# notu97/GS-SLAM-Analytica_Jacobian

Measured on AMD Instinct MI355X. Metric: Gaussian-pixel interactions/sec (fwd+Jacobian), 640x480, higher is better.
Workload: dtype f32; 1 GPU; cfg2: 50000 Gaussians (SH degree 3, 16 coeffs), 640x480; one step = one mapping window of 8 keyframes with distinct cameras: forward splat + analytical-Jacobian backward (dL/dmu, dL/dSigma->conic, per-Gaussian grads summed over the window, one dL/dtau per keyframe)

## Files before the change

gs-slam-analytica_jacobian_amd/csrc/api.hip:

```cpp
#include <stdarg.h>
#include <stdio.h>
#include <string.h>

#include <atomic>
#include <mutex>

#include "gsaj_common.h"
#include "loss_terms.h"

static thread_local char g_err[512] = "";

void gsaj_set_error(const char *fmt, ...) {
  va_list ap;
  va_start(ap, fmt);
  vsnprintf(g_err, sizeof(g_err), fmt, ap);
  va_end(ap);
}

struct ProfRec { int stage; hipEvent_t a, b; };
static std::mutex g_prof_mu;
static ProfRec *g_prof = nullptr;
static std::atomic<bool> g_prof_on{false};
static int g_prof_cap = 0;
static std::atomic<int> g_prof_n{0};
static thread_local int t_prof_open = -1;

void gsaj_prof_mark(int stage, int is_stop, hipStream_t s) {
  if (!g_prof_on.load(std::memory_order_acquire)) return;
  std::lock_guard<std::mutex> lk(g_prof_mu);
  if (!g_prof) return;
  if (!is_stop) {
    const int i = g_prof_n.fetch_add(1);
    if (i >= g_prof_cap) { g_prof_n.store(g_prof_cap); t_prof_open = -1; return; }
    t_prof_open = i;
    g_prof[i].stage = stage;
    (void)hipEventRecord(g_prof[i].a, s);
  } else if (t_prof_open >= 0 && t_prof_open < g_prof_cap) {
    (void)hipEventRecord(g_prof[t_prof_open].b, s);
    t_prof_open = -1;
  }
}

extern "C" {

int gsaj_profile_begin(int max_records) {
  std::lock_guard<std::mutex> lk(g_prof_mu);
  if (g_prof || max_records <= 0) {
    gsaj_set_error("gsaj_profile_begin: already active or bad size");
    return GSAJ_ERR_INVALID_ARGUMENT;
  }
  g_prof = new ProfRec[max_records];
  for (int i = 0; i < max_records; i++) {
    GSAJ_HIP_CHECK(hipEventCreate(&g_prof[i].a));
    GSAJ_HIP_CHECK(hipEventCreate(&g_prof[i].b));
  }
  g_prof_cap = max_records;
  g_prof_n.store(0);
  g_prof_on.store(true, std::memory_order_release);
  return GSAJ_OK;
}

int gsaj_profile_end(float *stage_ms, int *stage_launches) {
  if (!stage_ms || !stage_launches) {
    gsaj_set_error("gsaj_profile_end: null output");
    return GSAJ_ERR_INVALID_ARGUMENT;
  }
  g_prof_on.store(false, std::memory_order_release);
  GSAJ_HIP_CHECK(hipDeviceSynchronize());
  std::lock_guard<std::mutex> lk(g_prof_mu);
  if (!g_prof) {
    gsaj_set_error("gsaj_profile_end: not active");
    return GSAJ_ERR_INVALID_ARGUMENT;
  }
  for (int i = 0; i < ST_COUNT; i++) { stage_ms[i] = 0.f; stage_launches[i] = 0; }
  const int nrec = g_prof_n.load() < g_prof_cap ? g_prof_n.load() : g_prof_cap;
  for (int i = 0; i < nrec; i++) {
    float ms = 0.f;
    if (hipEventElapsedTime(&ms, g_prof[i].a, g_prof[i].b) == hipSuccess) {
      stage_ms[g_prof[i].stage] += ms;
      stage_launches[g_prof[i].stage] += 1;
    }
  }
  for (int i = 0; i < g_prof_cap; i++) { (void)hipEventDestroy(g_prof[i].a); (void)hipEventDestroy(g_prof[i].b); }
  delete[] g_prof;
  g_prof = nullptr;
  g_prof_cap = 0;
  g_prof_n.store(0);
  return GSAJ_OK;
}

const char *gsaj_last_error(void) { return g_err; }
int gsaj_version(void) { return 109; }

size_t gsaj_geom_workspace_bytes(int P) { return geom_carve(nullptr, (size_t)(P > 0 ? P : 0), nullptr) + 256; }
size_t gsaj_image_workspace_bytes(int W, int H) { return image_carve(nullptr, W, H, nullptr) + 256; }
size_t gsaj_binning_workspace_bytes(int R) {
  return bin_carve(nullptr, (size_t)(R > 0 ? R : 0), nullptr) + 256;
}

// ... 849 lines not shown
```

gs-slam-analytica_jacobian_amd/csrc/gaussian_bwd.hip:

```cpp
#include "gsaj_common.h"
#include "wave_reduce.h"
__constant__ float bSH_C0 = 0.28209479177387814f;
__constant__ float bSH_C1 = 0.4886025119029199f;
__constant__ float bSH_C2[5] = {1.0925484305920792f, -1.0925484305920792f, 0.31539156525252005f, -1.0925484305920792f,
                                0.5462742152960396f};
__constant__ float bSH_C3[7] = {-0.5900435899266435f, 2.890611442640554f, -0.4570457994644658f, 0.3731763325901154f,
                                -0.4570457994644658f, 1.445305721320277f, -0.5900435899266435f};
#define GSAJ_SH_CONSTANTS_DEFINED
#include "gaussian_chain.h"

__device__ __forceinline__ void gsaj_load_partials4(const float *p0, const float *p1, const float *p2, const float *p3,
                                                    float4 (&lo)[4], float4 (&hi)[4]) {
  asm volatile(
      "global_load_dwordx4 %0, %8, off sc0 sc1\n\tglobal_load_dwordx4 %1, %8, off offset:16 sc0 sc1\n\t"
      "global_load_dwordx4 %2, %9, off sc0 sc1\n\tglobal_load_dwordx4 %3, %9, off offset:16 sc0 sc1\n\t"
      "global_load_dwordx4 %4, %10, off sc0 sc1\n\tglobal_load_dwordx4 %5, %10, off offset:16 sc0 sc1\n\t"
      "global_load_dwordx4 %6, %11, off sc0 sc1\n\tglobal_load_dwordx4 %7, %11, off offset:16 sc0 sc1\n\t"
      "s_waitcnt vmcnt(0)"
      : "=&v"(lo[0]), "=&v"(hi[0]), "=&v"(lo[1]), "=&v"(hi[1]), "=&v"(lo[2]), "=&v"(hi[2]), "=&v"(lo[3]), "=&v"(hi[3])
      : "v"(p0), "v"(p1), "v"(p2), "v"(p3)
      : "memory");
}
__device__ __forceinline__ void gsaj_sum_partials(const float *partials, int nblk, int lane, double (&acc)[6]) {
  for (int i0 = lane; i0 < nblk; i0 += 4 * 64) {
// ... 540 lines not shown
        t6[k] = wave_sum<CW_G>(tau[k]);
      }
      if (gl == 0) {
        float4 *tp = reinterpret_cast<float4 *>(g.tau_partials + (size_t)blockIdx.x * 8);
        tp[0] = make_float4(t6[0], t6[1], t6[2], t6[3]);
        tp[1] = make_float4(t6[4], t6[5], 0.f, 0.f);
      }
    }
    float *mine = rowv + vl * NV * CW_G + gl;
    mine[0 * CW_G] = o.op; mine[1 * CW_G] = o.gm.x; mine[2 * CW_G] = o.gm.y; mine[3 * CW_G] = o.gm.z;
#pragma unroll
    for (int k = 0; k < 6; k++) mine[(4 + k) * CW_G] = o.cov[k];
    if constexpr (GATHER && SHW > 0) {
      if (!sh_left) {
        mine[10 * CW_G] = 0.f; mine[11 * CW_G] = 0.f; mine[12 * CW_G] = 0.f;
#pragma unroll
        for (int k = 0; k < MC; k++) mine[(13 + k) * CW_G] = 0.f;
      }
    } else {
      mine[10 * CW_G] = gmask.x; mine[11 * CW_G] = gmask.y; mine[12 * CW_G] = gmask.z;
#pragma unroll
      for (int k = 0; k < MC; k++) mine[(13 + k) * CW_G] = w[k];
    }
    __syncthreads();
    const int nv = min(CW_V, K - v0);
#pragma unroll
    for (int j = 0; j < EPT; j++) {
      const int e = tid + j * (CW_G * CW_V);
      const int c = e / CW_G;
      if (c < NE) {
        float sacc = acc[j];
        if (c < 10) {
#pragma unroll 2
          for (int u = 0; u < nv; u++) sacc += rowv[u * NV * CW_G + c * CW_G + gl];
        } else {
          const int kk = (c - 10) / 3, ch = (c - 10) - 3 * kk;
#pragma unroll 2
          for (int u = 0; u < nv; u++) sacc += rowv[u * NV * CW_G + (13 + kk) * CW_G + gl] * rowv[u * NV * CW_G + (10 + ch) * CW_G + gl];
        }
        acc[j] = sacc;
      }
    }
    __syncthreads();
  }
#pragma unroll
  for (int j = 0; j < EPT; j++) {
    const int e = tid + j * (CW_G * CW_V);
    if (e < NE * CW_G) outv[e] = acc[j];
  }
  __syncthreads();
#define OUT(dst, x) dst = accumulate ? dst + (x) : (x)
  const int nG = min(CW_G, p.P - (int)blockIdx.x * CW_G);
  const size_t b0 = (size_t)blockIdx.x * CW_G;
  for (int e = tid; e < nG; e += CW_G * CW_V) OUT(p.dL_dopacity[b0 + e], outv[0 * CW_G + e]);
  for (int e = tid; e < 3 * nG; e += CW_G * CW_V) OUT(p.dL_dmean3D[3 * b0 + e], outv[(1 + e % 3) * CW_G + e / 3]);
  for (int e = tid; e < 6 * nG; e += CW_G * CW_V) OUT(p.dL_dcov3D[6 * b0 + e], outv[(4 + e % 6) * CW_G + e / 6]);
  if (SHW > 0 && p.dL_dsh) {
    for (int e = tid; e < SHW * nG; e += CW_G * CW_V) OUT(p.dL_dsh[(size_t)SHW * b0 + e], outv[(10 + e % SHW) * CW_G + e / SHW]);
  }
  if (p.scales && tid < nG) {
    const size_t i = b0 + tid;
    float gcov[6];
#pragma unroll
    for (int k = 0; k < 6; k++) gcov[k] = outv[(4 + k) * CW_G + tid];
    const float3 sc = make_float3(p.scales[3 * i], p.scales[3 * i + 1], p.scales[3 * i + 2]);
    const float4 q = reinterpret_cast<const float4 *>(p.rotations)[i];
    float3 dscale;
    float4 drot;
    cov3d_backward(gcov, sc, q, p.scale_modifier, dscale, drot);
    OUT(p.dL_dscale[3 * i], dscale.x); OUT(p.dL_dscale[3 * i + 1], dscale.y); OUT(p.dL_dscale[3 * i + 2], dscale.z);
    float4 *dr = reinterpret_cast<float4 *>(p.dL_drot) + i;
    if (accumulate) { const float4 o4 = *dr; drot.x += o4.x; drot.y += o4.y; drot.z += o4.z; drot.w += o4.w; }
    *dr = drot;
  }
#undef OUT
  GSAJ_TRACE_END(gbb)
}

__global__ __launch_bounds__(256) void k_tau_sum(BwdParams p, GeomWS g0, ViewStrides vs) {
  __shared__ double red[256 * 6];
  const int tid = threadIdx.x, view = blockIdx.x, nslot = (p.P + CW_G - 1) / CW_G;
  const float4 *tp = reinterpret_cast<const float4 *>(gsaj_shift(g0.tau_partials, (size_t)view * vs.geom));
  double a[6] = {0.0, 0.0, 0.0, 0.0, 0.0, 0.0};
  for (int i = tid; i < nslot; i += 256) {
    const float4 lo = tp[2 * i], hi = tp[2 * i + 1];
    a[0] += (double)lo.x; a[1] += (double)lo.y; a[2] += (double)lo.z; a[3] += (double)lo.w; a[4] += (double)hi.x; a[5] += (double)hi.y;
  }
#pragma unroll
  for (int k = 0; k < 6; k++) red[k * 256 + tid] = a[k];
  __syncthreads();
  for (int o = 128; o > 0; o >>= 1) {
    if (tid < o) {
#pragma unroll
      for (int k = 0; k < 6; k++) red[k * 256 + tid] += red[k * 256 + tid + o];
    }
    __syncthreads();
  }
  if (tid < 6 && p.dL_dtau_sum) p.dL_dtau_sum[6 * view + tid] = (float)red[tid * 256];
}

template <int SHW, bool GATHER>
static void launch_chain(const BwdParams &p, int K, const GeomWS &g, const BinWS &b, const ImageWS &im, ViewStrides vs, int accumulate,
                         hipStream_t s) {
  for (int v0 = 0; v0 < K; v0 += CW_V)
    hipLaunchKernelGGL((k_chain_window<SHW, GATHER>), dim3((p.P + CW_G - 1) / CW_G), dim3(CW_G * CW_V), 0, s, p, v0, K, g, im, vs,
                       b.inst_grad, b.reached, p.dL_dmean2D, p.dL_dconic, p.dL_dcolor, p.dL_ddepth, p.dL_dtau,
                       (accumulate || v0 > 0) ? 1 : 0);
  hipLaunchKernelGGL(k_tau_sum, dim3(K), dim3(256), 0, s, p, g, vs);
}

int launch_gather_sums(int P, int K, const int *radii, const GeomWS &g, const BinWS &b, const ImageWS &im, ViewStrides vs, hipStream_t s) {
  GsajProfScope ps(ST_GATHER_SUMS, s);
  hipLaunchKernelGGL(k_gather_sums, dim3((P + 255) / 256, K), dim3(256), 0, s, P, radii, g, im, b.inst_grad, b.reached, vs);
  GSAJ_HIP_CHECK(hipGetLastError());
  return GSAJ_OK;
}

int launch_gaussian_backward_batch(const BwdParams &p, int K, const GeomWS &g, const BinWS &b, const ImageWS &im, ViewStrides vs,
                                   int accumulate, int gather, hipStream_t s) {
  GsajProfScope ps(ST_GAUSSIAN_BWD, s);
#define CHAIN(SHW)                                                       \
  if (gather) launch_chain<SHW, true>(p, K, g, b, im, vs, accumulate, s); \
  else launch_chain<SHW, false>(p, K, g, b, im, vs, accumulate, s);       \
  break
  switch (p.shs ? p.M : 0) {
    case 0: CHAIN(0);
    case 1: CHAIN(3);
    case 4: CHAIN(12);
    case 9: CHAIN(27);
    case 16: CHAIN(48);
    default:
      gsaj_set_error("batched backward: SH storage of %d coefficients is not supported (1, 4, 9 or 16)", p.M);
      return GSAJ_ERR_INVALID_ARGUMENT;
  }
#undef CHAIN
  GSAJ_HIP_CHECK(hipGetLastError());
  return GSAJ_OK;
}
```

gs-slam-analytica_jacobian_amd/csrc/gsaj_common.h:

```cpp
#pragma once
#include <hip/hip_runtime.h>
#include <stddef.h>
#include <stdint.h>

#include "../../include/gsaj.h"

#define GSAJ_WAVE 64
#define TILE GSAJ_TILE
#define TILE_PIXELS (TILE * TILE)
#define PRE_BLOCK 256
#define GB_BLOCK 64
#define REC_F4 3
#define IGRAD_F 12


static inline __host__ __device__ size_t gsaj_align(size_t x) { return (x + 255) & ~(size_t)255; }

struct GeomWS {
  float *depths;
  float *cov3D;
  uint8_t *clamped;
  uint32_t *tiles_touched;
  uint32_t *point_offsets;
  int *internal_radii;
  uint32_t *block_sums;
  float *tau_partials;
  float4 *splat;
  float4 *splat16;
  uint2 *scat;
  float4 *gsum;
};

static inline __host__ __device__ size_t geom_carve(char *base, size_t P, GeomWS *g) {
  size_t off = 0;
  size_t nblk = (P + PRE_BLOCK - 1) / PRE_BLOCK;
  if (nblk == 0) nblk = 1;
#define CARVE(field, type, count)                                \
  do {                                                           \
    if (g) g->field = reinterpret_cast<type *>(base + off);      \
    off += gsaj_align(sizeof(type) * (size_t)(count));           \
  } while (0)
  CARVE(depths, float, P);
  CARVE(cov3D, float, P * 6);
  CARVE(clamped, uint8_t, P * 3);
  CARVE(tiles_touched, uint32_t, P);
  CARVE(point_offsets, uint32_t, P);
  CARVE(internal_radii, int, P);
  CARVE(block_sums, uint32_t, nblk);
  CARVE(tau_partials, float, ((P + 31) / 32 + 1) * 8);
  CARVE(splat, float4, P * 3);
  CARVE(splat16, float4, P * 2);
  CARVE(scat, uint2, P);
  CARVE(gsum, float4, P * 3);
  return off;
}

#define TILE_REP 1
#define LDS_TILES_MAX 8192
#define SORT_CAP 16384
#define N_COUNTERS 64
#define ERR_PREFILTERED 1u
#define ERR_INTERNAL 2u
#define ERR_CAPACITY 4u
#define ERR_TILE_LIST 8u

struct ImageWS {
  float *final_T;
  uint32_t *n_contrib;
  uint2 *ranges;
  uint32_t *counters;
  uint32_t *tile_count;
  uint32_t *tile_cursor;
  uint32_t *tile_offset;
  uint32_t *sticky;
  uint32_t *tile_order;
  size_t zero_bytes;
};

static inline __host__ __device__ size_t image_carve(char *base, int W, int H, ImageWS *s) {
  size_t off = 0;
  size_t N = (size_t)W * H;
  size_t tiles = (size_t)((W + TILE - 1) / TILE) * ((H + TILE - 1) / TILE);
  ImageWS *g = s;
  CARVE(final_T, float, N);
  CARVE(n_contrib, uint32_t, N);
  CARVE(ranges, uint2, tiles);
  const size_t z0 = off;
  CARVE(counters, uint32_t, N_COUNTERS);
  CARVE(tile_count, uint32_t, tiles * TILE_REP);
  CARVE(tile_cursor, uint32_t, tiles * TILE_REP);
  if (g) g->zero_bytes = off - z0;
  CARVE(tile_offset, uint32_t, tiles * TILE_REP + 1);
  CARVE(sticky, uint32_t, 16);
  CARVE(tile_order, uint32_t, tiles);
  return off;
}

struct BinWS {
  uint64_t *keys_unsorted;
  uint64_t *keys;
  uint32_t *point_list;
  float4 *inst_grad;
  uint8_t *reached;
  uint32_t *taken;
};

struct ViewStrides {
  size_t geom, image, bin;
};
#ifdef __HIPCC__
#include <type_traits>
template <typename T>
__device__ __forceinline__ T *gsaj_shift(T *p, size_t bytes) {
  typedef typename std::conditional<std::is_const<T>::value, const char, char>::type byte_t;
  return reinterpret_cast<T *>(reinterpret_cast<byte_t *>(p) + bytes);
}
__device__ __forceinline__ GeomWS geom_view(GeomWS g, size_t off) {
  g.depths = gsaj_shift(g.depths, off); g.cov3D = gsaj_shift(g.cov3D, off); g.clamped = gsaj_shift(g.clamped, off);
  g.tiles_touched = gsaj_shift(g.tiles_touched, off); g.point_offsets = gsaj_shift(g.point_offsets, off);
  g.internal_radii = gsaj_shift(g.internal_radii, off); g.block_sums = gsaj_shift(g.block_sums, off);
  g.tau_partials = gsaj_shift(g.tau_partials, off); g.splat = gsaj_shift(g.splat, off); g.gsum = gsaj_shift(g.gsum, off);
  g.splat16 = gsaj_shift(g.splat16, off); g.scat = gsaj_shift(g.scat, off);
  return g;
}
__device__ __forceinline__ ImageWS image_view(ImageWS m, size_t off) {
  m.final_T = gsaj_shift(m.final_T, off); m.n_contrib = gsaj_shift(m.n_contrib, off); m.ranges = gsaj_shift(m.ranges, off);
  m.counters = gsaj_shift(m.counters, off); m.tile_count = gsaj_shift(m.tile_count, off);
  m.tile_cursor = gsaj_shift(m.tile_cursor, off); m.tile_offset = gsaj_shift(m.tile_offset, off);
  m.sticky = gsaj_shift(m.sticky, off); m.tile_order = gsaj_shift(m.tile_order, off);
  return m;
}
#endif

static inline size_t bin_carve(char *base, size_t R, BinWS *g) {
  size_t off = 0;
  size_t Rn = R ? R : 1;
  CARVE(keys_unsorted, uint64_t, Rn);
  CARVE(keys, uint64_t, Rn);
  CARVE(point_list, uint32_t, Rn);
  CARVE(inst_grad, float4, Rn * REC_F4);
  CARVE(reached, uint8_t, Rn);
  CARVE(taken, uint32_t, Rn);
  return off;
}
#undef CARVE

struct Carved { GeomWS g; BinWS b; ImageWS im; ViewStrides vs; };

void gsaj_set_error(const char *fmt, ...);
#define GSAJ_HIP_CHECK(expr)                                                          \
  do {                                                                                \
    hipError_t _e = (expr);                                                           \
    if (_e != hipSuccess) {                                                           \
      gsaj_set_error("%s failed: %s (%s:%d)", #expr, hipGetErrorString(_e), __FILE__, __LINE__); \
      return GSAJ_ERR_HIP;                                                            \
    }                                                                                 \
  } while (0)

enum GsajStage {
  ST_PREPROCESS = 0, ST_SCAN, ST_EMIT_KEYS, ST_SORT, ST_RANGES_RECORDS, ST_RENDER_FWD, ST_RENDER_BWD, ST_GAUSSIAN_BWD,
  ST_TAU_FINALIZE, ST_DENSE_BWD, ST_DENSE_REDUCE, ST_SCATTER, ST_TILE_SORT, ST_GATHER_SUMS, ST_COUNT
};
void gsaj_prof_mark(int stage, int is_stop, hipStream_t s);
struct GsajProfScope {
  int stage;
  hipStream_t s;
  GsajProfScope(int st, hipStream_t stream) : stage(st), s(stream) { gsaj_prof_mark(stage, 0, s); }
  ~GsajProfScope() { gsaj_prof_mark(stage, 1, s); }
};

struct FwdParams {
  int P, D, M, W, H;
  const float *means3D, *shs, *colors_precomp, *opacities, *scales, *rotations, *cov3D_precomp;
  const float *viewmatrix, *projmatrix, *campos;
  float scale_modifier, tanfovx, tanfovy, focal_x, focal_y;
  int prefiltered;
  int grid_x, grid_y;
  int capacity;
  int sort_cap;
  int bpw;
  int views;
};

int launch_preprocess(const FwdParams &p, int *radii, int *n_touched, const GeomWS &g, const ImageWS &im, ViewStrides vs,
                      hipStream_t s);
int launch_tile_binning(int P, int sort_cap, int rec16, int grid_x, int grid_y, const GeomWS &g, const BinWS &b, const ImageWS &im,
                        int views, ViewStrides vs, hipStream_t s);
struct FusedLoss;
int launch_render_forward(int P, int W, int H, int grid_x, int grid_y, const float *bg, const GeomWS &g, const BinWS &b,
                          const ImageWS &im, float *out_color, float *out_depth, float *out_opacity, int *n_touched, int views,
                          ViewStrides vs, hipStream_t s, const FusedLoss *fl = nullptr);
int gsaj_fwd_loss_slots(int W, int H);
int launch_loss_finalize(const FusedLoss &fl, int nslots, int W, int H, const uint32_t *aborted, float *out_scalars, hipStream_t s,
                         int views = 1, size_t abort_stride = 0, float *out_dexposure = nullptr);
int launch_render_backward(int R, int W, int H, int grid_x, int grid_y, const float *bg, const GeomWS &g, const BinWS &b,
                           const ImageWS &im, const float *dL_dpix, const float *dL_dpix_depth, int views, ViewStrides vs,
                           hipStream_t s, const FusedLoss *fl = nullptr);
int launch_export_taken(int W, int H, int grid_x, int grid_y, const BinWS &b, const ImageWS &im, uint32_t *out, hipStream_t s);
struct BwdParams {
  int P, D, M, W, H;
  const float *means3D, *shs, *scales, *rotations, *cov3Ds;
  const float *viewmatrix, *projmatrix, *projmatrix_raw, *campos;
  float scale_modifier, tanfovx, tanfovy, focal_x, focal_y;
  int grid_x, grid_y;
  const int *radii;
  float *dL_dmean2D, *dL_dconic, *dL_dopacity, *dL_dcolor, *dL_ddepth, *dL_dmean3D, *dL_dcov3D, *dL_dsh, *dL_dscale,
      *dL_drot, *dL_dtau, *dL_dtau_sum;
};
int launch_gaussian_backward(const BwdParams &p, const GeomWS &g, const BinWS &b, const ImageWS &im, hipStream_t s);
int launch_gather_sums(int P, int K, const int *radii, const GeomWS &g, const BinWS &b, const ImageWS &im, ViewStrides vs, hipStream_t s);
int launch_gaussian_backward_batch(const BwdParams &p, int K, const GeomWS &g, const BinWS &b, const ImageWS &im, ViewStrides vs,
                                   int accumulate, int gather, hipStream_t s);
size_t gsaj_jac_rows_bytes(int P);
int gsaj_jac_slots(int W, int H);
int launch_splat_jac(const BwdParams &p, const GeomWS &g, const ImageWS &im, float *rows, hipStream_t s);
struct JacOut {
  float *jac;
  float *color, *depth;
  const float *seed_c, *seed_d;
  const float *curv_c, *curv_d;
  float *partials;
  float delta;
};
int launch_render_jac(const BwdParams &p, const float *bg, const GeomWS &g, const BinWS &b, const ImageWS &im, const float *rows,
                      const JacOut &jo, const FusedLoss *fl, int joint, hipStream_t s);
int launch_gn_reduce(const float *partials, int n, const ImageWS &im, float *H_out, float *g_out, hipStream_t s);
int launch_splat_jac_batch(const BwdParams &p, int K, const GeomWS &g, const ImageWS &im, float *rows, ViewStrides vs, hipStream_t s);
int launch_render_jac_batch(const BwdParams &p, int K, const float *bg, const Carved &c, const float *rows, const JacOut &jo,
                            const FusedLoss &fl, int joint, hipStream_t s);
int launch_mark_visible(int P, const float *means3D, const float *viewmatrix, uint8_t *present, hipStream_t s);
void launch_exclusive_scan_u32(int n, uint32_t *v, hipStream_t s);
int launch_select_rank_f32(int W, int H, const float *values, uint32_t rank, uint32_t *out_key, void *seed_ws, hipStream_t s);

#ifdef __HIPCC__
__device__ __forceinline__ float3 xform4x3(const float *m, float3 p) {
  return make_float3(m[0] * p.x + m[4] * p.y + m[8] * p.z + m[12], m[1] * p.x + m[5] * p.y + m[9] * p.z + m[13],
                     m[2] * p.x + m[6] * p.y + m[10] * p.z + m[14]);
}
__device__ __forceinline__ float4 xform4x4(const float *m, float3 p) {
  return make_float4(m[0] * p.x + m[4] * p.y + m[8] * p.z + m[12], m[1] * p.x + m[5] * p.y + m[9] * p.z + m[13],
                     m[2] * p.x + m[6] * p.y + m[10] * p.z + m[14], m[3] * p.x + m[7] * p.y + m[11] * p.z + m[15]);
}
__device__ __forceinline__ float ndc2pix(float v, int S) { return (float)((((double)v + 1.0) * (double)S - 1.0) * 0.5); }

__device__ __forceinline__ uint32_t gsaj_tile_band(const uint32_t *__restrict__ sticky) {
  const uint32_t band = sticky[1];
  return sticky[2] == ~band ? band : 0u;
}
__device__ __forceinline__ void tile_rect(float px, float py, int r, int gx, int gy, uint32_t band, int &x0, int &y0, int &x1,
                                          int &y1) {
  const int ylo = band ? (int)(band & 0xffffu) : 0, yhi = band ? min(gy, (int)(band >> 16)) : gy;
  x0 = min(gx, max(0, (int)((px - (float)r) / (float)TILE)));
// ... 116 lines not shown
```

gs-slam-analytica_jacobian_amd/csrc/preprocess.hip:

```cpp
#include "gsaj_common.h"
#include "wave_reduce.h"

__constant__ float kSH_C0 = 0.28209479177387814f;
__constant__ float kSH_C1 = 0.4886025119029199f;
__constant__ float kSH_C2[5] = {1.0925484305920792f, -1.0925484305920792f, 0.31539156525252005f, -1.0925484305920792f,
                                0.5462742152960396f};
__constant__ float kSH_C3[7] = {-0.5900435899266435f, 2.890611442640554f, -0.4570457994644658f, 0.3731763325901154f,
                                -0.4570457994644658f, 1.445305721320277f, -0.5900435899266435f};

__device__ __forceinline__ float3 ld3(const float *p, size_t i) { return make_float3(p[3 * i], p[3 * i + 1], p[3 * i + 2]); }

__device__ __forceinline__ void cov3d_from_scale_rot(float3 sc, float mod, float4 q, float *c6) {
  const float r = q.x, x = q.y, y = q.z, z = q.w;
  float R[3][3] = {{1.f - 2.f * (y * y + z * z), 2.f * (x * y - r * z), 2.f * (x * z + r * y)},
                   {2.f * (x * y + r * z), 1.f - 2.f * (x * x + z * z), 2.f * (y * z - r * x)},
                   {2.f * (x * z - r * y), 2.f * (y * z + r * x), 1.f - 2.f * (x * x + y * y)}};
  const float s[3] = {mod * sc.x, mod * sc.y, mod * sc.z};
  float A[3][3];
#pragma unroll
  for (int i = 0; i < 3; i++)
#pragma unroll
    for (int j = 0; j < 3; j++) A[i][j] = s[i] * R[j][i];
  float S[3][3];
#pragma unroll
  for (int a = 0; a < 3; a++)
#pragma unroll
    for (int b = a; b < 3; b++) S[a][b] = A[0][a] * A[0][b] + A[1][a] * A[1][b] + A[2][a] * A[2][b];
  c6[0] = S[0][0]; c6[1] = S[0][1]; c6[2] = S[0][2]; c6[3] = S[1][1]; c6[4] = S[1][2]; c6[5] = S[2][2];
}

__device__ __forceinline__ float3 cov2d_forward(float3 mean, float fx, float fy, float tanx, float tany, const float *c6,
                                                const float *vm) {
  float3 t = xform4x3(vm, mean);
  const float limx = 1.3f * tanx, limy = 1.3f * tany;
  const float txtz = t.x / t.z, tytz = t.y / t.z;
  t.x = fminf(limx, fmaxf(-limx, txtz)) * t.z;
  t.y = fminf(limy, fmaxf(-limy, tytz)) * t.z;
  const float J00 = fx / t.z, J02 = -(fx * t.x) / (t.z * t.z);
  const float J11 = fy / t.z, J12 = -(fy * t.y) / (t.z * t.z);
  float M[2][3];
#pragma unroll
  for (int k = 0; k < 3; k++) {
    M[0][k] = vm[4 * k + 0] * J00 + vm[4 * k + 1] * 0.0f + vm[4 * k + 2] * J02;
    M[1][k] = vm[4 * k + 0] * 0.0f + vm[4 * k + 1] * J11 + vm[4 * k + 2] * J12;
  }
  const float V[3][3] = {{c6[0], c6[1], c6[2]}, {c6[1], c6[3], c6[4]}, {c6[2], c6[4], c6[5]}};
  float X[2][3];
#pragma unroll
  for (int r = 0; r < 2; r++)
#pragma unroll
    for (int c = 0; c < 3; c++) X[r][c] = M[r][0] * V[c][0] + M[r][1] * V[c][1] + M[r][2] * V[c][2];
  float3 cov;
  cov.x = (X[0][0] * M[0][0] + X[0][1] * M[0][1] + X[0][2] * M[0][2]) + 0.3f;
  cov.y = X[1][0] * M[0][0] + X[1][1] * M[0][1] + X[1][2] * M[0][2];
  cov.z = (X[1][0] * M[1][0] + X[1][1] * M[1][1] + X[1][2] * M[1][2]) + 0.3f;
  return cov;
}

__device__ __forceinline__ float3 sh_to_rgb(int deg, float3 pos, float3 campos, const float *sh, uint8_t *clamped) {
  float3 d = make_float3(pos.x - campos.x, pos.y - campos.y, pos.z - campos.z);
  const float len = sqrtf(d.x * d.x + d.y * d.y + d.z * d.z);
  const float x = d.x / len, y = d.y / len, z = d.z / len;
  float out[3];
#pragma unroll
  for (int ch = 0; ch < 3; ch++) {
#define SHC(k) sh[(k) * 3 + ch]
    float res = kSH_C0 * SHC(0);
    if (deg > 0) {
      res = res - kSH_C1 * y * SHC(1) + kSH_C1 * z * SHC(2) - kSH_C1 * x * SHC(3);
      if (deg > 1) {
        const float xx = x * x, yy = y * y, zz = z * z, xy = x * y, yz = y * z, xz = x * z;
        res = res + kSH_C2[0] * xy * SHC(4) + kSH_C2[1] * yz * SHC(5) + kSH_C2[2] * (2.0f * zz - xx - yy) * SHC(6) +
              kSH_C2[3] * xz * SHC(7) + kSH_C2[4] * (xx - yy) * SHC(8);
        if (deg > 2) {
          res = res + kSH_C3[0] * y * (3.0f * xx - yy) * SHC(9) + kSH_C3[1] * xy * z * SHC(10) +
                kSH_C3[2] * y * (4.0f * zz - xx - yy) * SHC(11) + kSH_C3[3] * z * (2.0f * zz - 3.0f * xx - 3.0f * yy) * SHC(12) +
                kSH_C3[4] * x * (4.0f * zz - xx - yy) * SHC(13) + kSH_C3[5] * z * (xx - yy) * SHC(14) +
                kSH_C3[6] * x * (xx - 3.0f * yy) * SHC(15);
        }
      }
    }
#undef SHC
    res += 0.5f;
    clamped[ch] = (res < 0.0f);
    out[ch] = res < 0.0f ? 0.0f : res;
  }
  return make_float3(out[0], out[1], out[2]);
}

GSAJ_TRACE_DEFINE(pre)

template <bool SH16, bool MULTI>
__global__ __launch_bounds__(PRE_BLOCK) void k_preprocess(FwdParams p, int *__restrict__ radii, int *__restrict__ n_touched,
                                                         GeomWS g, ImageWS im, ViewStrides vs) {
  __shared__ uint32_t scan[PRE_BLOCK / 64];
  extern __shared__ uint32_t hist[];
  {
    const size_t view = blockIdx.y;
    g = geom_view(g, view * vs.geom);
    im = image_view(im, view * vs.image);
    p.viewmatrix += 16 * view;
    p.projmatrix += 16 * view;
    if (p.campos) p.campos += 3 * view;
    radii += view * (size_t)p.P;
    n_touched += view * (size_t)p.P;
  }
  GSAJ_TRACE_BEGIN(pre)
#ifdef GSAJ_BLOCK_TRACE
  unsigned long long trp_[4] = {0, 0, 0, 0}, trp_t = wall_clock64();
#define TRP(i) { const unsigned long long n_ = wall_clock64(); trp_[i] += n_ - trp_t; trp_t = n_; }
#else
#define TRP(i)
#endif
  const int tid = threadIdx.x;
  const int tiles = p.grid_x * p.grid_y;
  const bool use_lds = tiles <= LDS_TILES_MAX;
  if (use_lds) {
    for (int t = tid; t < tiles; t += PRE_BLOCK) hist[t] = 0u;
    __syncthreads();
  }
  const int nblk_all = (p.P + PRE_BLOCK - 1) / PRE_BLOCK;
#pragma clang loop unroll(disable)
  for (int it = 0; it < (MULTI ? p.bpw : 1); it++) {
  const int blk = MULTI ? (int)blockIdx.x * p.bpw + it : (int)blockIdx.x;
  if (blk >= nblk_all) break;
  const int idx = blk * PRE_BLOCK + tid;
  uint32_t touched = 0;
  uint32_t rect_x = 0, rect_y = 0;
  float depth = 0.f;
  if (idx < p.P) {
    int my_radius_i = 0;
    uint32_t rect_pack = 0;
    float2 xy = make_float2(0.f, 0.f);
    float4 con_o = make_float4(0.f, 0.f, 0.f, 0.f);
    float3 rgb = make_float3(0.f, 0.f, 0.f);
    uint8_t cl[3] = {0, 0, 0};
    float c6s[6] = {0.f, 0.f, 0.f, 0.f, 0.f, 0.f};
    const float3 p_orig = ld3(p.means3D, idx);
    float3 sc_in = make_float3(0.f, 0.f, 0.f);
    float4 q_in = make_float4(1.f, 0.f, 0.f, 0.f);
    if (!p.cov3D_precomp) {
      sc_in = ld3(p.scales, idx);
      q_in = reinterpret_cast<const float4 *>(p.rotations)[idx];
    }
    const float opac_in = p.opacities[idx];
    constexpr bool sh_regs = SH16;
    float shv[SH16 ? 48 : 1];
    if (sh_regs) {
      const float4 *s4 = reinterpret_cast<const float4 *>(p.shs + (size_t)idx * 48);
#pragma unroll
      for (int k = 0; k < 12; k++) {
        const float4 t = s4[k];
        shv[4 * k] = t.x; shv[4 * k + 1] = t.y; shv[4 * k + 2] = t.z; shv[4 * k + 3] = t.w;
      }
    }
    const float3 p_view = xform4x3(p.viewmatrix, p_orig);
    if (p_view.z <= 0.2f) {
      if (p.prefiltered) atomicOr(&im.counters[1], ERR_PREFILTERED);
    } else {
      const float4 p_hom = xform4x4(p.projmatrix, p_orig);
      const float p_w = 1.0f / (p_hom.w + 0.0000001f);
      const float3 p_proj = make_float3(p_hom.x * p_w, p_hom.y * p_w, p_hom.z * p_w);
      float c6[6];
      if (p.cov3D_precomp) {
#pragma unroll
        for (int k = 0; k < 6; k++) c6[k] = p.cov3D_precomp[6 * (size_t)idx + k];
      } else {
        cov3d_from_scale_rot(sc_in, p.scale_modifier, q_in, c6s);
#pragma unroll
        for (int k = 0; k < 6; k++) c6[k] = c6s[k];
      }
      const float3 cov = cov2d_forward(p_orig, p.focal_x, p.focal_y, p.tanfovx, p.tanfovy, c6, p.viewmatrix);
      const float det = cov.x * cov.z - cov.y * cov.y;
      if (det != 0.0f) {
        const float det_inv = 1.f / det;
        const float3 conic = make_float3(cov.z * det_inv, -cov.y * det_inv, cov.x * det_inv);
        const float mid = 0.5f * (cov.x + cov.z);
        const float sq = sqrtf(fmaxf(0.1f, mid * mid - det));
        const float lambda1 = mid + sq, lambda2 = mid - sq;
        const float my_radius = ceilf(3.f * sqrtf(fmaxf(lambda1, lambda2)));
        const float2 pim = make_float2(ndc2pix(p_proj.x, p.W), ndc2pix(p_proj.y, p.H));
        int x0, y0, x1, y1;
        tile_rect(pim.x, pim.y, (int)my_radius, p.grid_x, p.grid_y, gsaj_tile_band(im.sticky), x0, y0, x1, y1);
        const int area = (x1 - x0) * (y1 - y0);
        if (area != 0) {
          if (!p.colors_precomp) {
            const float3 cam = make_float3(p.campos[0], p.campos[1], p.campos[2]);
            if constexpr (sh_regs) rgb = sh_to_rgb(p.D, p_orig, cam, shv, cl);
            else rgb = sh_to_rgb(p.D, p_orig, cam, p.shs + (size_t)idx * p.M * 3, cl);
          }
          rect_pack = (uint32_t)x0 | ((uint32_t)y0 << 10) | ((uint32_t)(x1 - x0) << 20);
          rect_x = (uint32_t)x0 | ((uint32_t)x1 << 16);
          rect_y = (uint32_t)y0 | ((uint32_t)y1 << 16);
          depth = p_view.z;
          my_radius_i = (int)my_radius;
          xy = pim;
          con_o = make_float4(conic.x, conic.y, conic.z, opac_in);
          touched = (uint32_t)area;
          for (int y = y0; y < y1; y++)
            for (int x = x0; x < x1; x++) {
              if (use_lds) atomicAdd(&hist[y * p.grid_x + x], 1u);
              else atomicAdd(&im.tile_count[y * p.grid_x + x], 1u);
            }
        }
      }
    }
    radii[idx] = my_radius_i;
    n_touched[idx] = 0;
    g.depths[idx] = depth;
    if (!p.cov3D_precomp && blockIdx.y == 0) {
#pragma unroll
      for (int k = 0; k < 6; k++) g.cov3D[6 * (size_t)idx + k] = c6s[k];
    }
    if (!p.colors_precomp) {
      g.clamped[3 * (size_t)idx] = cl[0]; g.clamped[3 * (size_t)idx + 1] = cl[1]; g.clamped[3 * (size_t)idx + 2] = cl[2];
    }
    g.tiles_touched[idx] = touched;
    if (p.colors_precomp) rgb = ld3(p.colors_precomp, idx);
    g.splat[3 * (size_t)idx + 0] = make_float4(xy.x, xy.y, __uint_as_float(rect_pack), 0.f);
    g.splat[3 * (size_t)idx + 1] = con_o;
    g.splat[3 * (size_t)idx + 2] = make_float4(rgb.x, rgb.y, rgb.z, depth);
  }
  TRP(0)
  const uint32_t first = block_excl_scan_add<PRE_BLOCK / 64>(touched, scan);
  if (idx < p.P) {
    g.point_offsets[idx] = first + touched;
    reinterpret_cast<float *>(g.splat)[12 * (size_t)idx + 3] = __uint_as_float(first);
    g.scat[idx] = make_uint2(rect_x, rect_y);
  }
  if (tid == 0) g.block_sums[blk] = block_scan_total<PRE_BLOCK / 64>(scan);
  __syncthreads();
  }
  if (use_lds)
    for (int t = tid; t < tiles; t += PRE_BLOCK) {
      const uint32_t c = hist[t];
      if (c) atomicAdd(&im.tile_count[t], c);
    }
  TRP(1)
  GSAJ_TRACE_END(pre)
#ifdef GSAJ_BLOCK_TRACE
  if ((threadIdx.x & 63) == 0) {
    unsigned long long *t = g_trace_pre + 4 * (blockIdx.x * (PRE_BLOCK / 64) + (threadIdx.x >> 6));
    t[2] = (trp_[0] << 32) | trp_[1];
    t[3] = 0;
  }
#endif
}

__device__ uint32_t tile_scan_and_schedule(int tiles, ImageWS im, uint32_t *len, uint32_t *longest_out) {
  __shared__ uint32_t wsum[PRE_BLOCK / 64], wmax[PRE_BLOCK / 64], cls[64];
  const int tid = threadIdx.x;
  for (int c = tid; 4 * c < tiles; c += PRE_BLOCK) {
    const uint4 v = *reinterpret_cast<const uint4 *>(im.tile_count + 4 * c);
    len[4 * c] = v.x;
    if (4 * c + 1 < tiles) len[4 * c + 1] = v.y;
    if (4 * c + 2 < tiles) len[4 * c + 2] = v.z;
    if (4 * c + 3 < tiles) len[4 * c + 3] = v.w;
  }
  if (tid < 64) cls[tid] = 0u;
  __syncthreads();
  uint32_t longest;
  const uint32_t total = block_excl_scan_runs<PRE_BLOCK / 64>(len, im.tile_offset, tiles, wsum, wmax, longest);
  const int shift = longest >= 64u ? (32 - __builtin_clz(longest)) - 6 : 0;
  for (int t = tid; t < tiles; t += PRE_BLOCK) atomicAdd(&cls[63u - min(63u, len[t] >> shift)], 1u);
  __syncthreads();
  if (tid < 64) {
    const uint32_t v = cls[tid];
    cls[tid] = wave_incl_scan_add(v) - v;
  }
  __syncthreads();
  for (int t = tid; t < tiles; t += PRE_BLOCK) im.tile_order[atomicAdd(&cls[63u - min(63u, len[t] >> shift)], 1u)] = (uint32_t)t;
  __syncthreads();
  *longest_out = longest;
  return total;
}

__global__ __launch_bounds__(PRE_BLOCK) void k_frame_scan(int nblk, int tiles, int capacity, GeomWS g, ImageWS im, ViewStrides vs) {
  extern __shared__ uint32_t lds_len[];
  g = geom_view(g, (size_t)blockIdx.y * vs.geom);
  im = image_view(im, (size_t)blockIdx.y * vs.image);
  __shared__ uint32_t wsum[PRE_BLOCK / 64], wmax[PRE_BLOCK / 64];
  uint32_t *block_sums = g.block_sums;
  uint32_t m, R2;
  const uint32_t R = block_excl_scan_runs<PRE_BLOCK / 64>(block_sums, block_sums, nblk, wsum, wmax, m);
  __syncthreads();
  if (tiles <= LDS_TILES_MAX) {
    R2 = tile_scan_and_schedule(tiles, im, lds_len, &m);
  } else {
    R2 = block_excl_scan_runs<PRE_BLOCK / 64>(im.tile_count, im.tile_offset, tiles, wsum, wmax, m);
    for (int t = threadIdx.x; t < tiles; t += PRE_BLOCK) im.tile_order[t] = (uint32_t)t;
  }
  if (threadIdx.x == 0) {
    im.tile_offset[tiles] = R2;
    im.counters[0] = R;
    im.counters[2] = m;
    uint32_t err = 0u;
    if (R2 != R) err |= ERR_INTERNAL;
    if (capacity > 0) {
      if (R > (uint32_t)capacity) err |= ERR_CAPACITY;
      if (err) {
        im.counters[4] = 1u;
        atomicAdd(&im.sticky[0], 1u);
      }
    }
    if (err) atomicOr(&im.counters[1], err);
  }
}

#ifndef SCAT_CLS
#define SCAT_CLS 8
#endif
#define SCAT_LDS_TILES 4096
#define SCAT_STAGE 4096
GSAJ_TRACE_DEFINE(scat)

__global__ __launch_bounds__(PRE_BLOCK) void k_scatter_instances(int P, int gx, int gy, int gpt, GeomWS g, ImageWS im,
                                                                 uint32_t *__restrict__ inst_id, ViewStrides vs) {
  extern __shared__ uint32_t lds[];
  __shared__ uint32_t stage_id[SCAT_STAGE];
  __shared__ uint16_t stage_lt[SCAT_STAGE];
  __shared__ uint32_t s_wave[PRE_BLOCK / 64], s_carry;
  {
    const size_t view = blockIdx.y;
    g = geom_view(g, view * vs.geom);
    im = image_view(im, view * vs.image);
    inst_id = gsaj_shift(inst_id, view * vs.bin);
  }
  if (im.counters[4]) return;
  GSAJ_TRACE_BEGIN(scat)
#ifdef GSAJ_BLOCK_TRACE
  unsigned long long trs_[4] = {0, 0, 0, 0}, trs_t = wall_clock64();
#define TRS(i) { const unsigned long long n_ = wall_clock64(); trs_[i] += n_ - trs_t; trs_t = n_; }
#else
#define TRS(i)
#endif
  const int tid = threadIdx.x;
  const int cls = (int)(blockIdx.x % SCAT_CLS), gb = (int)(blockIdx.x / SCAT_CLS);
  const int rows_c = (gy - cls + SCAT_CLS - 1) / SCAT_CLS;
  const int ltiles = rows_c > 0 ? rows_c * gx : 0;
  const bool use_lds = ((gy + SCAT_CLS - 1) / SCAT_CLS) * gx <= SCAT_LDS_TILES;
  uint32_t *cnt = lds, *fill = lds + ltiles, *lbase = lds + 2 * ltiles;
  if (use_lds) {
    for (int t = tid; t < 2 * ltiles; t += PRE_BLOCK) lds[t] = 0u;
    if (tid == 0) s_carry = 0u;
    __syncthreads();
  }
#define SCAT_FOR_EACH_TILE(BODY)                                                                     \
  for (int i0 = 0; i0 < gpt; i0 += 4) {                                                              \
    uint2 sc[4];                                                                                     \
    _Pragma("unroll") for (int j = 0; j < 4; j++) {                                                  \
      const int idx = (gb * gpt + i0 + j) * PRE_BLOCK + tid;                                         \
      sc[j] = (i0 + j < gpt && idx < P) ? g.scat[idx] : make_uint2(0u, 0u);                          \
    }                                                                                                \
    _Pragma("unroll") for (int j = 0; j < 4; j++) {                                                  \
      const int x0 = (int)(sc[j].x & 0xffffu), x1 = (int)(sc[j].x >> 16);                            \
      const int y0 = (int)(sc[j].y & 0xffffu), y1 = (int)(sc[j].y >> 16);                            \
      if (x1 > x0) {                                                                                 \
        const uint32_t id = (uint32_t)((gb * gpt + i0 + j) * PRE_BLOCK + tid);                       \
        (void)id;                                                                                    \
        const int ys = y0 + ((cls - y0) % SCAT_CLS + SCAT_CLS) % SCAT_CLS;                           \
        for (int y = ys; y < y1; y += SCAT_CLS)                                                      \
          for (int x = x0; x < x1; x++) {                                                            \
            const int lt = (y / SCAT_CLS) * gx + x;                            \
            const int t = y * gx + x;                                                      \
            (void)lt; (void)t;                                                                       \
            BODY                                                                                     \
          }                                                                                          \
      }                                                                                              \
    }                                                                                                \
  }
  if (!use_lds) {
    SCAT_FOR_EACH_TILE({ inst_id[im.tile_offset[t] + atomicAdd(&im.tile_cursor[t], 1u)] = id; })
    return;
  }
  TRS(0)
  SCAT_FOR_EACH_TILE({ atomicAdd(&cnt[lt], 1u); })
  __syncthreads();
  TRS(1)
  for (int l0 = 0; l0 < ltiles; l0 += PRE_BLOCK) {
    const int lt = l0 + tid;
    uint32_t c = 0u, off = 0u, base = 0u;
    if (lt < ltiles) {
      const int j = lt / gx;
      const int t = (j * SCAT_CLS + cls) * gx + (lt - j * gx);
      c = cnt[lt];
      off = im.tile_offset[t];
      if (c) base = atomicAdd(&im.tile_cursor[t], c);
    }
// ... 262 lines not shown
    }
    __syncthreads();
    lds_bitonic_sort<NT>(lds, T, tid);
    for (int i = tid; i < len; i += NT) b[c0 + i] = lds[i];
    __syncthreads();
  }
  uint64_t *src = b, *dst = a;
  for (long long width = T; width < (long long)n; width <<= 1) {
    asm volatile("s_waitcnt vmcnt(0)" ::: "memory");
    __syncthreads();
    for (long long p0 = 0; p0 < (long long)n; p0 += 2 * width) {
      const int la = (int)min(width, (long long)n - p0);
      const int lb = (int)max(0ll, min(width, (long long)n - p0 - width));
      const uint64_t *A = src + p0, *B = src + p0 + width;
      uint64_t *D = dst + p0;
      if (lb == 0) {
        for (int i = tid; i < la; i += NT) D[i] = A[i];
        continue;
      }
      const int tot = la + lb, nblk = (tot + T - 1) / T;
      for (int j0 = 0; j0 < nblk; j0 += PRE_BLOCK) {
        for (int t = tid; t <= PRE_BLOCK; t += NT) {
          const long long dl = (long long)(j0 + t) * T;
          const int d = (int)min(dl, (long long)tot);
          int lo = max(0, d - lb), hi = min(d, la);
          while (lo < hi) {
            const int mid = (lo + hi) >> 1;
            if (A[mid] <= B[d - 1 - mid]) lo = mid + 1;
            else hi = mid;
          }
          split_s[t] = (uint32_t)lo;
        }
        __syncthreads();
        for (int j = j0; j < min(nblk, j0 + PRE_BLOCK); j++) {
          const int a0 = (int)split_s[j - j0], a1 = (int)split_s[j - j0 + 1];
          const int d0 = j * T, d1 = min(tot, d0 + T);
          const int b0 = d0 - a0, cA = a1 - a0, cB = (d1 - a1) - b0;
          for (int i = tid; i < T; i += NT) lds[i] = i < cA ? A[a0 + i] : (i >= T - cB ? B[b0 + (T - 1 - i)] : KEY_INF);
          __syncthreads();
          lds_bitonic_merge<NT>(lds, T, tid);
          for (int i = tid; i < cA + cB; i += NT) D[d0 + i] = lds[i];
          __syncthreads();
        }
      }
    }
    uint64_t *t = src;
    src = dst;
    dst = t;
  }
  asm volatile("s_waitcnt vmcnt(0)" ::: "memory");
  __syncthreads();
  return src;
}

GSAJ_TRACE_DEFINE(sort)

#ifndef GSAJ_SORT_128_MAX
#define GSAJ_SORT_128_MAX 1024
#endif
template <int NT>
__global__ __launch_bounds__(NT) void k_tile_sort(ImageWS im, const float *__restrict__ depths, uint64_t *__restrict__ inst_key,
                                                   uint64_t *__restrict__ keys_b, uint32_t *point_list,
                                                   uint8_t *__restrict__ reached, int cap, int pass, int rec16, ViewStrides vs) {
  {
    const size_t view = blockIdx.y;
    im = image_view(im, view * vs.image);
    depths = gsaj_shift(depths, view * vs.geom);
    inst_key = gsaj_shift(inst_key, view * vs.bin);
    keys_b = gsaj_shift(keys_b, view * vs.bin);
    point_list = gsaj_shift(point_list, view * vs.bin);
    reached = gsaj_shift(reached, view * vs.bin);
  }
  extern __shared__ uint64_t keys[];
  if (im.counters[4]) return;
  GSAJ_TRACE_BEGIN(sort)
#ifdef GSAJ_BLOCK_TRACE
  unsigned long long tr_a = wall_clock64(), tr_b = 0, tr_c = 0;
#endif
  const int tid = threadIdx.x, tile = blockIdx.x;
  const uint32_t beg = im.tile_offset[tile * TILE_REP], end = im.tile_offset[(tile + 1) * TILE_REP];
  const int n = (int)(end - beg);
  if (pass != 2) {
    if (tid == 0) im.ranges[tile] = n > 0 ? make_uint2(beg, end) : make_uint2(0u, 0u);
    if (tid == 0 && tile == 0) im.counters[7] = (uint32_t)rec16;
    for (uint32_t k = beg + tid; k < end; k += NT) reached[k] = 0;
  }
  if (n == 0) return;
  const uint64_t *sorted = keys;
  if (n > cap) {
    if (pass == 2) return;
    const int T = cap >= 4096 ? cap / 2 : cap;
    sorted = sort_long_list<NT>(keys, T, reinterpret_cast<uint32_t *>(keys + T), point_list + beg, depths, inst_key + beg, keys_b + beg, n, tid);
  } else {
    int m = 2;
    while (m < n) m <<= 1;
    if (pass == 1 && 2 * m <= cap) return;
    if (pass == 2 && m > cap) return;
    const int nup = ((n + 127) >> 7) << 7;
    for (int i0 = tid; i0 < nup; i0 += 4 * NT) {
      uint32_t id[4], dz[4];
#pragma unroll
      for (int u = 0; u < 4; u++) id[u] = point_list[beg + (uint32_t)min(i0 + u * NT, n - 1)];
#pragma unroll
      for (int u = 0; u < 4; u++) dz[u] = __float_as_uint(depths[id[u]]);
#pragma unroll
      for (int u = 0; u < 4; u++) asm volatile("" : "+v"(dz[u]));
#pragma unroll
      for (int u = 0; u < 4; u++) {
        const int i = i0 + u * NT;
        if (i < nup) keys[i] = i < n ? ((uint64_t)dz[u] << 32) | id[u] : KEY_INF;
      }
    }
    __syncthreads();
#ifdef GSAJ_BLOCK_TRACE
    tr_b = wall_clock64();
#endif
    lds_bitonic_sort<NT>(keys, n, tid);
  }
#ifdef GSAJ_BLOCK_TRACE
  tr_c = wall_clock64();
#endif
  for (int i = tid; i < n; i += NT) point_list[beg + (uint32_t)i] = (uint32_t)sorted[i];
  GSAJ_TRACE_END(sort)
#ifdef GSAJ_BLOCK_TRACE
  if ((threadIdx.x & 63) == 0) {
    unsigned long long *t = g_trace_sort + 4 * (blockIdx.x * (NT / 64) + (threadIdx.x >> 6));
    t[2] = tr_b - tr_a;
    t[3] = tr_c - tr_b;
  }
#endif
}

__global__ __launch_bounds__(PRE_BLOCK) void k_mark_visible(int P, const float *__restrict__ means3D,
                                                            const float *__restrict__ vm, uint8_t *__restrict__ present) {
  const int idx = blockIdx.x * PRE_BLOCK + threadIdx.x;
  if (idx >= P) return;
  const float3 pv = xform4x3(vm, ld3(means3D, idx));
  present[idx] = pv.z > 0.2f;
}

__global__ __launch_bounds__(256) void k_zero_frame_state(uint32_t *__restrict__ counters, size_t words, size_t view_stride) {
  uint32_t *c = gsaj_shift(counters, blockIdx.y * view_stride);
  for (size_t i = (size_t)blockIdx.x * 256 + threadIdx.x; i < words; i += (size_t)gridDim.x * 256) c[i] = 0u;
}

int launch_preprocess(const FwdParams &p0, int *radii, int *n_touched, const GeomWS &g, const ImageWS &im, ViewStrides vs,
                      hipStream_t s) {
  FwdParams p = p0;
  const int nblk = (p.P + PRE_BLOCK - 1) / PRE_BLOCK;
  const int views = p.views > 0 ? p.views : 1;
  p.bpw = 1;
  while (p.bpw < 8 && (long long)nblk * views / (2 * p.bpw) >= 4096) p.bpw *= 2;
  const int nwg = (nblk + p.bpw - 1) / p.bpw;
  {
    const size_t words = im.zero_bytes / sizeof(uint32_t);
    hipLaunchKernelGGL(k_zero_frame_state, dim3((unsigned)((words + 1023) / 1024), views), dim3(256), 0, s, im.counters, words,
                       vs.image);
  }
  {
    GsajProfScope ps(ST_PREPROCESS, s);
    const int tiles = p.grid_x * p.grid_y;
    const size_t lds = tiles <= LDS_TILES_MAX ? sizeof(uint32_t) * (size_t)tiles : 0;
#ifndef GSAJ_PRE_NO_SHREGS
    if (!p.colors_precomp && p.M == 16)
#else
    if (false)
#endif
      if (p.bpw > 1) hipLaunchKernelGGL((k_preprocess<true, true>), dim3(nwg, views), dim3(PRE_BLOCK), lds, s, p, radii, n_touched, g, im, vs);
      else hipLaunchKernelGGL((k_preprocess<true, false>), dim3(nwg, views), dim3(PRE_BLOCK), lds, s, p, radii, n_touched, g, im, vs);
    else
      if (p.bpw > 1) hipLaunchKernelGGL((k_preprocess<false, true>), dim3(nwg, views), dim3(PRE_BLOCK), lds, s, p, radii, n_touched, g, im, vs);
      else hipLaunchKernelGGL((k_preprocess<false, false>), dim3(nwg, views), dim3(PRE_BLOCK), lds, s, p, radii, n_touched, g, im, vs);
    hipLaunchKernelGGL(k_frame_scan, dim3(1, views), dim3(PRE_BLOCK), lds, s, nblk, tiles, p.capacity, g, im, vs);
  }
  GSAJ_HIP_CHECK(hipGetLastError());
  return GSAJ_OK;
}

int launch_tile_binning(int P, int sort_cap, int rec16, int grid_x, int grid_y, const GeomWS &g, const BinWS &b, const ImageWS &im,
                        int views, ViewStrides vs, hipStream_t s) {
  {
    GsajProfScope ps(ST_SCATTER, s);
    const int ltiles = ((grid_y + SCAT_CLS - 1) / SCAT_CLS) * grid_x;
    const size_t lds = ltiles <= SCAT_LDS_TILES ? 3 * sizeof(uint32_t) * (size_t)ltiles : 0;
    int gpt = 4;
    while (gpt < 8 && (long long)P * views * SCAT_CLS / ((long long)PRE_BLOCK * gpt * 2) >= 1536) gpt *= 2;
    for (int g2 = 9; gpt == 8 && g2 <= 10; g2++) {
      const long long wg8 = (long long)((P + PRE_BLOCK * 8 - 1) / (PRE_BLOCK * 8)) * SCAT_CLS * views;
      const long long wg2 = (long long)((P + PRE_BLOCK * g2 - 1) / (PRE_BLOCK * g2)) * SCAT_CLS * views;
      if (wg8 > 1536 && wg2 <= 1536) gpt = g2;
    }
    const int per = PRE_BLOCK * gpt;
    hipLaunchKernelGGL(k_scatter_instances, dim3((unsigned)((P + per - 1) / per) * SCAT_CLS, views), dim3(PRE_BLOCK), lds, s, P, grid_x,
                       grid_y, gpt, g, im, b.point_list, vs);
    if (rec16)
      hipLaunchKernelGGL(k_pack_splat16, dim3((P + 255) / 256, views), dim3(256), 0, s, P, g, im.counters, vs);
  }
  {
    GsajProfScope ps(ST_TILE_SORT, s);
    int cap = 128;
    while (cap < sort_cap && cap < SORT_CAP) cap <<= 1;
    if (sizeof(uint64_t) * (size_t)cap > 65536)
      (void)hipFuncSetAttribute(reinterpret_cast<const void *>(&k_tile_sort<512>), hipFuncAttributeMaxDynamicSharedMemorySize,
                                (int)(sizeof(uint64_t) * (size_t)cap));
    const size_t split_bytes = cap >= 4096 ? 0 : sizeof(uint32_t) * (PRE_BLOCK + 1);
    auto launch = [&](int lds_keys, int pass, size_t extra) {
      const size_t dyn = sizeof(uint64_t) * (size_t)lds_keys + extra;
      if (lds_keys >= 4096)
        hipLaunchKernelGGL(k_tile_sort<512>, dim3(grid_x * grid_y, views), dim3(512), dyn, s, im, g.depths, b.keys_unsorted, b.keys,
                           b.point_list, b.reached, lds_keys, pass, rec16, vs);
      else if (lds_keys > GSAJ_SORT_128_MAX)
        hipLaunchKernelGGL(k_tile_sort<256>, dim3(grid_x * grid_y, views), dim3(256), dyn, s, im, g.depths, b.keys_unsorted, b.keys,
                           b.point_list, b.reached, lds_keys, pass, rec16, vs);
      else
        hipLaunchKernelGGL(k_tile_sort<128>, dim3(grid_x * grid_y, views), dim3(128), dyn, s, im, g.depths, b.keys_unsorted, b.keys,
                           b.point_list, b.reached, lds_keys, pass, rec16, vs);
    };
    if (cap >= 4096) {
      launch(cap, 1, 0);
      launch(cap / 2, 2, 0);
    } else {
      launch(cap, 0, split_bytes);
    }
  }
  GSAJ_HIP_CHECK(hipGetLastError());
  return GSAJ_OK;
}

int launch_mark_visible(int P, const float *means3D, const float *viewmatrix, uint8_t *present, hipStream_t s) {
  const int nblk = (P + PRE_BLOCK - 1) / PRE_BLOCK;
  hipLaunchKernelGGL(k_mark_visible, dim3(nblk), dim3(PRE_BLOCK), 0, s, P, means3D, viewmatrix, present);
  GSAJ_HIP_CHECK(hipGetLastError());
  return GSAJ_OK;
}
```

Baseline: 718.9 billion interactions/s.

## Skip per-frame state zeroing by self-cleaning counters in scan and sort kernels

The consuming kernels now reset per-frame state themselves: frame_scan clears tile_count and rewrites the error and abort counters, and tile_sort clears tile_cursor. A host-side map records which frame-state buffers are known to be clean, so the k_zero_frame_state launch can be skipped on eager (non-captured) streams unless an environment override forces it. The tau reduction is also unrolled 8x so more loads are in flight per thread. The risk is correctness: the host tracking has to match what the device actually cleared, and any counter that is not self-reset would carry stale values into the next frame.

```diff
diff --git a/gs-slam-analytica_jacobian_amd/csrc/api.hip b/gs-slam-analytica_jacobian_amd/csrc/api.hip
--- a/gs-slam-analytica_jacobian_amd/csrc/api.hip
+++ b/gs-slam-analytica_jacobian_amd/csrc/api.hip
@@ -1,5 +1,6 @@
 #include <stdarg.h>
 #include <stdio.h>
+#include <stdlib.h>
 #include <string.h>
 
 #include <atomic>
@@ -15,6 +16,11 @@
   va_start(ap, fmt);
   vsnprintf(g_err, sizeof(g_err), fmt, ap);
   va_end(ap);
+}
+
+bool gsaj_reset_every_frame() {
+  const char *e = getenv("GSAJ_RESET_EVERY_FRAME");
+  return e && e[0] == '1';
 }
 
 struct ProfRec { int stage; hipEvent_t a, b; };
diff --git a/gs-slam-analytica_jacobian_amd/csrc/gaussian_bwd.hip b/gs-slam-analytica_jacobian_amd/csrc/gaussian_bwd.hip
--- a/gs-slam-analytica_jacobian_amd/csrc/gaussian_bwd.hip
+++ b/gs-slam-analytica_jacobian_amd/csrc/gaussian_bwd.hip
@@ -646,9 +646,20 @@
   const int tid = threadIdx.x, view = blockIdx.x, nslot = (p.P + CW_G - 1) / CW_G;
   const float4 *tp = reinterpret_cast<const float4 *>(gsaj_shift(g0.tau_partials, (size_t)view * vs.geom));
   double a[6] = {0.0, 0.0, 0.0, 0.0, 0.0, 0.0};
-  for (int i = tid; i < nslot; i += 256) {
-    const float4 lo = tp[2 * i], hi = tp[2 * i + 1];
-    a[0] += (double)lo.x; a[1] += (double)lo.y; a[2] += (double)lo.z; a[3] += (double)lo.w; a[4] += (double)hi.x; a[5] += (double)hi.y;
+  for (int i0 = tid; i0 < nslot; i0 += 8 * 256) {
+    float4 lo[8], hi[8];
+#pragma unroll
+    for (int u = 0; u < 8; u++) {
+      const int i = min(i0 + u * 256, nslot - 1);
+      lo[u] = tp[2 * i];
+      hi[u] = tp[2 * i + 1];
+    }
+#pragma unroll
+    for (int u = 0; u < 8; u++)
+      if (i0 + u * 256 < nslot) {
+        a[0] += (double)lo[u].x; a[1] += (double)lo[u].y; a[2] += (double)lo[u].z; a[3] += (double)lo[u].w;
+        a[4] += (double)hi[u].x; a[5] += (double)hi[u].y;
+      }
   }
 #pragma unroll
   for (int k = 0; k < 6; k++) red[k * 256 + tid] = a[k];
diff --git a/gs-slam-analytica_jacobian_amd/csrc/gsaj_common.h b/gs-slam-analytica_jacobian_amd/csrc/gsaj_common.h
--- a/gs-slam-analytica_jacobian_amd/csrc/gsaj_common.h
+++ b/gs-slam-analytica_jacobian_amd/csrc/gsaj_common.h
@@ -59,6 +59,7 @@
 #define LDS_TILES_MAX 8192
 #define SORT_CAP 16384
 #define N_COUNTERS 64
+#define CNT_PRE_ERR 5
 #define ERR_PREFILTERED 1u
 #define ERR_INTERNAL 2u
 #define ERR_CAPACITY 4u
@@ -168,6 +169,8 @@
   GsajProfScope(int st, hipStream_t stream) : stage(st), s(stream) { gsaj_prof_mark(stage, 0, s); }
   ~GsajProfScope() { gsaj_prof_mark(stage, 1, s); }
 };
+
+bool gsaj_reset_every_frame();
 
 struct FwdParams {
   int P, D, M, W, H;
diff --git a/gs-slam-analytica_jacobian_amd/csrc/preprocess.hip b/gs-slam-analytica_jacobian_amd/csrc/preprocess.hip
--- a/gs-slam-analytica_jacobian_amd/csrc/preprocess.hip
+++ b/gs-slam-analytica_jacobian_amd/csrc/preprocess.hip
@@ -1,3 +1,6 @@
+#include <mutex>
+#include <unordered_map>
+
 #include "gsaj_common.h"
 #include "wave_reduce.h"
 
@@ -156,7 +159,7 @@
     }
     const float3 p_view = xform4x3(p.viewmatrix, p_orig);
     if (p_view.z <= 0.2f) {
-      if (p.prefiltered) atomicOr(&im.counters[1], ERR_PREFILTERED);
+      if (p.prefiltered) atomicOr(&im.counters[CNT_PRE_ERR], ERR_PREFILTERED);
     } else {
       const float4 p_hom = xform4x4(p.projmatrix, p_orig);
       const float p_w = 1.0f / (p_hom.w + 0.0000001f);
@@ -269,7 +272,10 @@
     cls[tid] = wave_incl_scan_add(v) - v;
   }
   __syncthreads();
-  for (int t = tid; t < tiles; t += PRE_BLOCK) im.tile_order[atomicAdd(&cls[63u - min(63u, len[t] >> shift)], 1u)] = (uint32_t)t;
+  for (int t = tid; t < tiles; t += PRE_BLOCK) {
+    im.tile_order[atomicAdd(&cls[63u - min(63u, len[t] >> shift)], 1u)] = (uint32_t)t;
+    im.tile_count[t] = 0u;
+  }
   __syncthreads();
   *longest_out = longest;
   return total;
@@ -281,6 +287,8 @@
   im = image_view(im, (size_t)blockIdx.y * vs.image);
   __shared__ uint32_t wsum[PRE_BLOCK / 64], wmax[PRE_BLOCK / 64];
   uint32_t *block_sums = g.block_sums;
+  uint32_t pre = 0u;
+  if (threadIdx.x == 0) pre = atomicExch(&im.counters[CNT_PRE_ERR], 0u);
   uint32_t m, R2;
   const uint32_t R = block_excl_scan_runs<PRE_BLOCK / 64>(block_sums, block_sums, nblk, wsum, wmax, m);
   __syncthreads();
@@ -288,22 +296,27 @@
     R2 = tile_scan_and_schedule(tiles, im, lds_len, &m);
   } else {
     R2 = block_excl_scan_runs<PRE_BLOCK / 64>(im.tile_count, im.tile_offset, tiles, wsum, wmax, m);
-    for (int t = threadIdx.x; t < tiles; t += PRE_BLOCK) im.tile_order[t] = (uint32_t)t;
+    __syncthreads();
+    for (int t = threadIdx.x; t < tiles; t += PRE_BLOCK) {
+      im.tile_order[t] = (uint32_t)t;
+      im.tile_count[t] = 0u;
+    }
   }
   if (threadIdx.x == 0) {
     im.tile_offset[tiles] = R2;
     im.counters[0] = R;
     im.counters[2] = m;
-    uint32_t err = 0u;
+    uint32_t err = 0u, abort = 0u;
     if (R2 != R) err |= ERR_INTERNAL;
     if (capacity > 0) {
       if (R > (uint32_t)capacity) err |= ERR_CAPACITY;
       if (err) {
-        im.counters[4] = 1u;
+        abort = 1u;
         atomicAdd(&im.sticky[0], 1u);
       }
     }
-    if (err) atomicOr(&im.counters[1], err);
+    im.counters[4] = abort;
+    im.counters[1] = pre | err;
   }
 }
 
@@ -732,6 +745,7 @@
   const int n = (int)(end - beg);
   if (pass != 2) {
     if (tid == 0) im.ranges[tile] = n > 0 ? make_uint2(beg, end) : make_uint2(0u, 0u);
+    if (tid == 0) im.tile_cursor[tile * TILE_REP] = 0u;
     if (tid == 0 && tile == 0) im.counters[7] = (uint32_t)rec16;
     for (uint32_t k = beg + tid; k < end; k += NT) reached[k] = 0;
   }
@@ -794,6 +808,27 @@
   for (size_t i = (size_t)blockIdx.x * 256 + threadIdx.x; i < words; i += (size_t)gridDim.x * 256) c[i] = 0u;
 }
 
+static std::mutex g_clean_mu;
+static std::unordered_map<const void *, size_t> g_clean;
+
+static bool frame_state_known_clean(const ImageWS &im, int views, size_t stride) {
+  std::lock_guard<std::mutex> lk(g_clean_mu);
+  for (int v = 0; v < views; v++) {
+    auto it = g_clean.find(reinterpret_cast<const char *>(im.counters) + (size_t)v * stride);
+    if (it == g_clean.end() || it->second != im.zero_bytes) return false;
+  }
+  return true;
+}
+static void frame_state_mark(const ImageWS &im, int views, size_t stride, bool clean) {
+  std::lock_guard<std::mutex> lk(g_clean_mu);
+  for (int v = 0; v < views; v++) {
+    const void *key = reinterpret_cast<const char *>(im.counters) + (size_t)v * stride;
+    if (clean) g_clean[key] = im.zero_bytes;
+    else g_clean.erase(key);
+  }
+  if (g_clean.size() > 4096) g_clean.clear();
+}
+
 int launch_preprocess(const FwdParams &p0, int *radii, int *n_touched, const GeomWS &g, const ImageWS &im, ViewStrides vs,
                       hipStream_t s) {
   FwdParams p = p0;
@@ -802,11 +837,14 @@
   p.bpw = 1;
   while (p.bpw < 8 && (long long)nblk * views / (2 * p.bpw) >= 4096) p.bpw *= 2;
   const int nwg = (nblk + p.bpw - 1) / p.bpw;
-  {
+  hipStreamCaptureStatus capture = hipStreamCaptureStatusNone;
+  const bool eager = hipStreamIsCapturing(s, &capture) == hipSuccess && capture == hipStreamCaptureStatusNone;
+  if (!(p.capacity > 0 && eager && !gsaj_reset_every_frame() && frame_state_known_clean(im, views, vs.image))) {
     const size_t words = im.zero_bytes / sizeof(uint32_t);
     hipLaunchKernelGGL(k_zero_frame_state, dim3((unsigned)((words + 1023) / 1024), views), dim3(256), 0, s, im.counters, words,
                        vs.image);
   }
+  frame_state_mark(im, views, vs.image, false);
   {
     GsajProfScope ps(ST_PREPROCESS, s);
     const int tiles = p.grid_x * p.grid_y;
@@ -824,11 +862,14 @@
     hipLaunchKernelGGL(k_frame_scan, dim3(1, views), dim3(PRE_BLOCK), lds, s, nblk, tiles, p.capacity, g, im, vs);
   }
   GSAJ_HIP_CHECK(hipGetLastError());
+  if (eager) frame_state_mark(im, views, vs.image, true);
   return GSAJ_OK;
 }
 
 int launch_tile_binning(int P, int sort_cap, int rec16, int grid_x, int grid_y, const GeomWS &g, const BinWS &b, const ImageWS &im,
                         int views, ViewStrides vs, hipStream_t s) {
+  const bool was_clean = frame_state_known_clean(im, views, vs.image);
+  frame_state_mark(im, views, vs.image, false);
   {
     GsajProfScope ps(ST_SCATTER, s);
     const int ltiles = ((grid_y + SCAT_CLS - 1) / SCAT_CLS) * grid_x;
@@ -874,6 +915,7 @@
     }
   }
   GSAJ_HIP_CHECK(hipGetLastError());
+  if (was_clean) frame_state_mark(im, views, vs.image, true);
   return GSAJ_OK;
 }
 
```

Result: no change. 719.4 billion interactions/s (median of 3 runs) (+0.1%).
